# ElenaRyumina/AVCER

Hardware: AMD Instinct MI355X
Metric: clips/sec (224x224x16f + 2s@16kHz), full AV path: static CNN + LSTM + wav2vec2 audio model + fusion (higher is better)
Workload: dtype f16x3 (f16 MFMA on hi/lo-split f32 operands, f32 accumulate)

## Files before the change

avcer_amd/_lib.py:

```python
from __future__ import annotations

import ctypes as C
import os

from .build import LIB, source_hash

c_ctx = C.c_void_p
c_stream = C.c_void_p


class ConvDesc(C.Structure):
    _fields_ = [
        ("batch", C.c_int32), ("in_h", C.c_int32), ("in_w", C.c_int32),
        ("out_h", C.c_int32), ("out_w", C.c_int32),
        ("cin", C.c_int32), ("kh", C.c_int32), ("kw", C.c_int32),
        ("stride_h", C.c_int32), ("stride_w", C.c_int32), ("pad_h", C.c_int32), ("pad_w", C.c_int32),
        ("dil_h", C.c_int32), ("dil_w", C.c_int32),
        ("x_stride_b", C.c_int64), ("x_stride_h", C.c_int64), ("x_stride_w", C.c_int64),
        ("x_coff", C.c_int32), ("n", C.c_int32),
        ("y_ld", C.c_int64), ("y_coff", C.c_int32),
        ("r_ld", C.c_int64), ("r_coff", C.c_int32),
        ("act", C.c_int32), ("res_after_act", C.c_int32), ("groups", C.c_int32),
        ("x2_cin", C.c_int32), ("x2_coff", C.c_int32), ("x2_stride", C.c_int32),
        ("x2_stride_b", C.c_int64), ("x2_stride_h", C.c_int64), ("x2_stride_w", C.c_int64),
# ... 62 lines not shown
    "avcer_cam_render": (C.c_int, [c_ctx, C.c_void_p, C.c_void_p, C.c_void_p, C.c_void_p, C.c_int, C.c_void_p, C.c_double,
                                   C.c_void_p, c_stream]),
    "avcer_fuse": (C.c_int, [c_ctx, C.c_void_p, C.c_void_p, C.c_void_p, C.c_int, C.c_int, C.c_int, C.c_void_p,
                             C.c_void_p, C.c_int, C.c_int, C.c_void_p, C.c_void_p, c_stream]),
    "avcer_conv_gemm": (C.c_int, [c_ctx, C.POINTER(ConvDesc), C.c_int, C.c_void_p, C.c_void_p, C.c_void_p, C.c_void_p,
                                  C.c_void_p, C.c_void_p, c_stream]),
    "avcer_split_weights": (C.c_int, [c_ctx, C.c_void_p, C.c_void_p, C.c_size_t, c_stream]),
    "avcer_split_weight_rows": (C.c_int, [c_ctx, C.c_void_p, C.c_void_p, C.c_int, C.c_int, c_stream]),
    "avcer_weight_frags": (C.c_int, [c_ctx, C.c_void_p, C.c_void_p, C.c_int, C.c_int, c_stream]),
    "avcer_conv_gemm_dual": (C.c_int, [c_ctx, C.POINTER(ConvDesc), C.c_int, C.c_void_p, C.c_void_p, C.c_void_p, C.c_void_p,
                                       C.c_void_p, C.c_void_p, C.c_void_p, c_stream]),
    "avcer_face_nms": (C.c_int, [c_ctx, C.c_void_p, C.c_int, C.c_int, C.c_float, C.c_float, C.c_int, C.c_int, C.c_float,
                                 C.c_void_p, C.c_void_p, c_stream]),
    "avcer_bneck_chain": (C.c_int, [c_ctx, C.c_int, C.c_int, C.c_int, C.c_int, C.c_void_p, C.c_void_p, C.c_int, C.c_int] + [C.c_void_p] * 9 +
                          [c_stream]),
    "avcer_stem_pool": (C.c_int, [c_ctx, C.c_void_p, C.c_size_t, C.c_void_p, C.c_void_p, C.c_void_p, C.c_void_p, C.c_int, c_stream]),
    "avcer_stem_pool_u8": (C.c_int, [c_ctx, C.c_void_p, C.c_int, C.c_int, C.c_int, C.c_void_p, C.c_void_p, C.c_void_p, C.c_void_p,
                                     c_stream]),
    "avcer_attention": (C.c_int, [c_ctx, C.c_void_p, C.c_void_p, C.c_int, C.c_int, C.c_int, C.c_int, C.c_float, C.c_int, C.c_int,
                                  c_stream]),
    "avcer_measure_ceilings": (C.c_int, [c_ctx, C.POINTER(C.c_double), C.POINTER(C.c_double), c_stream]),
    "avcer_gemm_stats": (C.c_int, [c_ctx, C.POINTER(C.c_int64), C.POINTER(C.c_double), C.c_int]),
    "avcer_profile_enable": (C.c_int, [c_ctx, C.c_int]),
    "avcer_profile_read": (C.c_int, [c_ctx, C.POINTER(C.c_double), C.POINTER(C.c_int64)]),
    "avcer_profile_read_families": (C.c_int, [c_ctx, C.c_int, C.POINTER(C.c_double), C.POINTER(C.c_int64), C.POINTER(C.c_double),
                                              C.POINTER(C.c_double)]),
    "avcer_profile_read_launches": (C.c_int, [c_ctx, C.c_int64, C.c_void_p, C.c_void_p, C.c_void_p, C.c_void_p, C.c_void_p,
                                              C.POINTER(C.c_int64)]),
    "avcer_debug_tap": (C.c_int, [c_ctx, C.c_char_p, C.c_void_p, C.c_size_t]),
    "avcer_debug_tap_copied": (C.c_int64, [c_ctx]),
# ... 44 lines not shown
```

avcer_amd/csrc/api.hip:

```cpp
#include "common.h"
#include "split_dev.h"
#include "_source_hash.h"

#include <algorithm>
#include <cmath>
#include <new>

int set_err(avcer_ctx* ctx, int code, const char* fmt, ...) {
    if (ctx) {
        va_list ap;
        va_start(ap, fmt);
        vsnprintf(ctx->err, sizeof(ctx->err), fmt, ap);
        va_end(ap);
    }
    return code;
}

int ws_reserve(avcer_ctx* ctx, int slot, size_t bytes, void** out) {
    DevBuf& b = ctx->ws[slot];
    if (b.cap < bytes) {
        if (b.p) {
            HIP_TRY(ctx, hipDeviceSynchronize());
            HIP_TRY(ctx, hipFree(b.p));
            b.p = nullptr;
// ... 398 lines not shown
    }
    return AVCER_OK;
}
extern "C" int avcer_audio_num_classes(const avcer_ctx* ctx) { return ctx ? ctx->aud_classes : 0; }
extern "C" int avcer_audio_head_kind(const avcer_ctx* ctx) { return ctx && ctx->aud.loaded ? ctx->aud_head : 0; }

struct Trunk {
    void* X;
    void* pp[2];
    void* T1;
    void* T2;
    int h, w, cin;
    bool stride_last;
    bool w2_frags;
    const char* tap;
};

static void run_bneck_stage(Net& net, Trunk& t, int li, int b_begin, int b_end, int nb, void* last_out, const std::string& end_tap) {
    avcer_ctx* ctx = net.ctx;
    const std::string tap = t.tap;
    const int act = net.act.kind;
    const size_t es = net.act.es;
    const int planes = kStages[li][0], blocks = kStages[li][1];
    const int fused_from = li == 0 ? 0 : 1;
    for (int b = b_begin; b < b_end; ++b) {
        const int s = t.stride_last ? (b == blocks - 1 && li < 3 ? kStages[li + 1][2] : 1) : (b == 0 ? kStages[li][2] : 1);
        const int h = t.h, w = t.w, oh = (h - 1) / s + 1, ow = (w - 1) / s + 1;
        const long M = (long)nb * h * w;
        const std::string p = "l" + std::to_string(li + 1) + "." + std::to_string(b) + ".",
                          pn = "l" + std::to_string(li + 1) + "." + std::to_string(b + 1) + ".";
        void* dst = (b == b_end - 1 && last_out) ? last_out : (t.X == t.pp[0] ? t.pp[1] : t.pp[0]);
        const bool fused = net.x3 && li < 3 && b >= fused_from, chain = fused && li < 2, next = b + 1 < blocks;
        if (!fused || b == fused_from)
            net.gemm(conv2d_desc(nb, h, w, t.cin, 1, 1, 1, 0, planes, 1), p + "c1.w", net.F(p + "c1.s"), net.F(p + "c1.b"), t.X,
                     nullptr, t.T1, act, act);
        if (chain) {
            const bool first = b == 0;
            const Tensor *w2 = net.T(p + "c2.wf"), *w3 = net.T(first ? p + "c3d.w" : p + "c3.wf"),
                         *w1n = next ? net.T(pn + "c1.wf") : nullptr;
            if (net.err != AVCER_OK) return;
            if (!w2->x3 || !w3->x3 || (next && !w1n->x3)) {
                net.err = set_err(ctx, AVCER_ESTATE, "%s: split chain weights not prepared", p.c_str());
                return;
            }
            net.chk(launch_bneck(ctx, planes, nb, h, w, t.T1, t.X, first ? t.cin : 0, s, dst, next ? t.T2 : nullptr, w2->x3,
                                 net.F(p + "c2.b"), w3->x3, net.F(first ? p + "c3d.b" : p + "c3.b"), next ? w1n->x3 : nullptr,
                                 next ? net.F(pn + "c1.b") : nullptr, net.st, t.w2_frags ? w2->x3f : nullptr));
            if (ctx->tap_dst) {
                net.tap((tap + "chain_out:" + p).c_str(), dst, (size_t)nb * oh * ow * planes * 4 * es);
                if (next) net.tap((tap + "chain_t1n:" + p).c_str(), t.T2, (size_t)M * planes * es);
            }
            std::swap(t.T1, t.T2);
        } else {
            net.gemm(conv2d_desc(nb, h, w, planes, 3, 3, s, 1, planes, 1), p + "c2.w", net.F(p + "c2.s"), net.F(p + "c2.b"), t.T1,
                     nullptr, t.T2, act, act);
            avcer_conv_desc d3 = conv2d_desc(nb, oh, ow, planes, 1, 1, 1, 0, planes * 4, 1);
            if (fused && next && M <= kTailPairRows) {
                net.gemm(d3, p + "c3.wf", nullptr, net.F(p + "c3.b"), t.T2, t.X, dst, act, act);
                net.gemm(conv2d_desc(nb, h, w, planes * 4, 1, 1, 1, 0, planes, 1), pn + "c1.wf", nullptr, net.F(pn + "c1.b"), dst,
                         nullptr, t.T1, act, act);
            } else if (fused && next) {
                const Tensor *w3 = net.T(p + "c3.wf"), *w1n = net.T(pn + "c1.wf");
                if (net.err != AVCER_OK) return;
                if (!w3->x3 || !w1n->x3) {
                    net.err = set_err(ctx, AVCER_ESTATE, "%s: split tail weights not prepared", p.c_str());
// ... 770 lines not shown
                                    avcer_stream_t stream) {
    if (!ctx || !d || !x2) return AVCER_EINVAL;
    HIP_TRY(ctx, hipSetDevice(ctx->device));
    return launch_conv_gemm(ctx, *d, dtype, x, w, scale, bias, residual, y, (hipStream_t)stream, x2);
}

extern "C" int avcer_bneck_chain(avcer_ctx* ctx, int planes, int nb, int h, int w, const void* t1, const void* x, int ds_cin,
                                 int out_step, void* out, void* t1n, const void* w2, const float* b2, const void* w3, const float* b3,
                                 const void* w1n, const float* b1n, const void* w2_frags, avcer_stream_t stream) {
    if (!ctx) return AVCER_EINVAL;
    if (nb <= 0 || h <= 0 || w <= 0) return set_err(ctx, AVCER_EINVAL, "bneck_chain: bad geometry");
    HIP_TRY(ctx, hipSetDevice(ctx->device));
    return launch_bneck(ctx, planes, nb, h, w, t1, x, ds_cin, out_step, out, t1n, w2, b2, w3, b3, w1n, b1n, (hipStream_t)stream, w2_frags);
}

extern "C" int avcer_stem_pool(avcer_ctx* ctx, const void* planes_hi_lo, size_t plane_bytes, const void* w, const float* scale,
                               const float* bias, void* y, int n, avcer_stream_t stream) {
    if (!ctx) return AVCER_EINVAL;
    if (plane_bytes != (size_t)n * 230 * 230 * 4 * 2) return set_err(ctx, AVCER_EINVAL, "stem_pool: plane_bytes != n*230*230*4*2");
    HIP_TRY(ctx, hipSetDevice(ctx->device));
    return launch_stem_pool(ctx, planes_hi_lo, plane_bytes, w, scale, bias, y, n, (hipStream_t)stream);
}

extern "C" int avcer_stem_pool_u8(avcer_ctx* ctx, const uint8_t* frames, int n, int in_h, int in_w, const void* w, const float* scale,
                                  const float* shifts9, void* y, avcer_stream_t stream) {
    if (!ctx) return AVCER_EINVAL;
    HIP_TRY(ctx, hipSetDevice(ctx->device));
    return launch_stem_pool_u8(ctx, frames, in_h, in_w, w, scale, shifts9, y, n, (hipStream_t)stream);
}

// ... 46 lines not shown
```

avcer_amd/csrc/common.h:

```cpp
#pragma once

#include <hip/hip_runtime.h>

#include <cstdarg>
#include <cstdint>
#include <cstdio>
#include <cstring>
#include <map>
#include <string>
#include <vector>

#include "../../include/avcer_hip.h"
#include "arena.h"

typedef uint16_t bf16_t;

struct DevBuf {
    void* p = nullptr;
    size_t cap = 0;
};

enum { WS_STATIC = 0, WS_DYNAMIC = 1, WS_AUDIO = 2, WS_FACE = 3, WS_NMS = 4, WS_CEILINGS = 5, WS_STATIC_LANE1 = 6, WS_FACE_LANE1 = 7,
       WS_GRU = 8, WS_COUNT = 9 };

// ... 80 lines not shown
int launch_stem_pool(avcer_ctx* ctx, const void* planes, size_t plane_bytes, const void* w_x3, const float* scale,
                     const float* bias, void* y, int n, hipStream_t st);
int launch_stem_pool_u8(avcer_ctx* ctx, const uint8_t* frames, int in_h, int in_w, const void* w_x3, const float* scale,
                        const float* bias9, void* y, int n, hipStream_t st);
int launch_stem_pool_face(avcer_ctx* ctx, const uint8_t* frames, int h, int w, int rgb, const void* w_x3, const float* scale,
                          const float* bias, void* y, int n, hipStream_t st);
inline double grid_rounds(long tiles, long slots) {
    const long whole = tiles / slots, rest = tiles % slots;
    if (whole == 0) return 2 * tiles <= slots ? 0.62 : 1.0;
    const double f = (double)rest / (double)slots;
    return (double)whole + (rest == 0 ? 0.0 : (2 * rest <= slots ? 0.25 + 0.7 * f : 1.0));
}

int launch_bneck(avcer_ctx* ctx, int planes, int nb, int h, int w, const void* t1, const void* x, int ds_cin, int out_step,
                 void* out, void* t1n, const void* w2, const float* b2, const void* w3, const float* b3, const void* w1n,
                 const float* b1n, hipStream_t st, const void* w2_frags = nullptr);

int launch_bneck_tail(avcer_ctx* ctx, int planes, long M, const void* t2, const void* x, void* out, void* t1n, const void* w3,
                      const float* b3, const void* w1n, const float* b1n, hipStream_t st);

int launch_gru_layer(avcer_ctx* ctx, const float* xp, const void* w, int x3, const float* bhh, int n, int S, float* h_seq, void* h_sp,
                     hipStream_t st);

int measure_ceilings(avcer_ctx* ctx, double* mfma_bf16_tflops, double* hbm_copy_tbs, hipStream_t st);

int k_preprocess(avcer_ctx*, const uint8_t* frames, int n, int in_h, int in_w, void* out, int kind, hipStream_t);
int k_maxpool3s2(avcer_ctx*, const void* x, void* y, int n, int h, int w, int c, int oh, int ow, int kind, hipStream_t);
int k_avgpool_hw(avcer_ctx*, const void* x, float* y, void* y_sp32, int n, int hw, int c, int kind, hipStream_t);
int k_cam_maps(avcer_ctx*, const void* x, const float* probs, const float* h, const float* w1, const float* w2, float* g,
               float* cam, int n, int kind, hipStream_t);
int k_small_linear(avcer_ctx*, const float* x, const float* w, const float* b, float* logits, float* probs, int m,
// ... 38 lines not shown
```

avcer_amd/csrc/fused.hip:

```cpp
#include "common.h"
#include "gemm_dev.h"

#include <algorithm>

namespace {

__device__ __forceinline__ void mfma3(f32x4_t& acc, const spx8_t wh, const spx8_t wl, const spx8_t ah, const spx8_t al) {
    acc = mfma_sp(wl, ah, acc);
    acc = mfma_sp(wh, al, acc);
    acc = mfma_sp(wh, ah, acc);
}

template <int A, int B>
__device__ __forceinline__ void pin(f32x4_t (&acc)[A][B]) {
#pragma unroll
    for (int a = 0; a < A; ++a)
#pragma unroll
        for (int b = 0; b < B; ++b) asm volatile("" : "+v"(acc[a][b]));
}
template <int A>
__device__ __forceinline__ void pin(f32x4_t (&acc)[A]) {
#pragma unroll
    for (int a = 0; a < A; ++a) asm volatile("" : "+v"(acc[a]));
}
// ... 368 lines not shown
    char* OUT;
    char* T1N;
    const char* W2;
    const char* W2F;
    const char* W3;
    const char* W1N;
    const float *b2, *b3, *b1n;
    unsigned t1_bytes;
    int M, H, Wd;
    int OH, OW;
    unsigned* ovf;
    int nblocks;
};

template <int P, int BM, bool NEXT, int NQX, bool PATCH, int SUB = 1, bool T11 = false>
__global__ void __launch_bounds__(256, P == 64 ? 3 : 2) bneck_kernel(const BneckParams p) {
    static_assert(SUB == 1 || (SUB == 2 && !NEXT && NQX == 0 && !PATCH), "the strided form is the plain last block of a stage");
    static_assert(!T11 || (P == 64 && BM == 128 && !PATCH && SUB == 1), "the spatial-tile form serves planes 64 at full resolution");
    constexpr int NQ = P / 32;
    constexpr int NQT = NQ + NQX;
    constexpr int PSLOTS = PATCH ? (P == 64 ? 456 : 304) : 0;
    constexpr int T11_E = 11, T11_PW = T11_E + 2, T11_SLOTS = 176;
    constexpr int NT = BM / 64;
    constexpr int NG = 4 * P / 32;
    constexpr int TILE_A = (BM + P) * ROWB;
    constexpr int TILE_B = (32 * NQT + P) * ROWB;
    constexpr int PHASE_A = T11 ? NQ * T11_SLOTS * ROWB : (PATCH ? PSLOTS * ROWB + 2 * P * ROWB : 2 * TILE_A);
    constexpr int TILES = PHASE_A > 2 * TILE_B ? PHASE_A : 2 * TILE_B;
    constexpr int NBIAS = 6 * P;
    __shared__ __attribute__((aligned(16))) char smem[TILES + NBIAS * 4];
    float* sbias = reinterpret_cast<float*>(smem + TILES);
    for (int i = threadIdx.x; i < NBIAS; i += 256)
        sbias[i] = i < P ? p.b2[i] : (i < 2 * P ? (NEXT ? p.b1n[i - P] : 0.f) : p.b3[i - 2 * P]);
    const int wave = __builtin_amdgcn_readfirstlane((int)threadIdx.x >> 6);
    sp_flags_t ovm = 0;
    const int tid = threadIdx.x, lane = tid & 63;
    const int g = lane >> 4, l15 = lane & 15;
    const int lrow8 = lane >> 3, slot = lane & 7;
    const int blk = xcd_remap(blockIdx.x, gridDim.x);
    const int m_base = blk * BM;
    const int t11_b = T11 ? blk / 25 : 0, t11_y0 = T11 ? ((blk % 25) / 5) * T11_E : 0, t11_x0 = T11 ? (blk % 5) * T11_E : 0;
    auto row_pos = [&](int r, bool& ok) -> int {
        if constexpr (T11) {
            ok = r < T11_E * T11_E;
            const int rr = ok ? r : T11_E * T11_E - 1;
            const int ry = rr / T11_E, rx = rr - ry * T11_E;
            return (t11_b * 55 + t11_y0 + ry) * 55 + t11_x0 + rx;
        } else {
            const long m = (long)m_base + r;
            ok = m < p.M;
            return ok ? (int)m : 0;
        }
    };

    const float s2 = split_wmul(p.W2, P * 9 * P * 4), s3 = split_wmul(p.W3, 4 * P * (P + 32 * NQX) * 4);
    const float s1n = NEXT ? split_wmul(p.W1N, 4 * P * P * 4) : 1.f;
    (void)s1n;
    const auto t1rs = __builtin_amdgcn_make_buffer_rsrc(const_cast<char*>(p.T1), (short)0, (int)p.t1_bytes, 0x00020000);
    const auto w2rs = __builtin_amdgcn_make_buffer_rsrc(const_cast<char*>(p.W2), (short)0, P * 9 * P * 4, 0x00020000);
    const auto w3rs = __builtin_amdgcn_make_buffer_rsrc(const_cast<char*>(p.W3), (short)0, 4 * P * (P + 32 * NQX) * 4, 0x00020000);
    const auto w1rs = __builtin_amdgcn_make_buffer_rsrc(const_cast<char*>(NEXT ? p.W1N : p.W3), (short)0, 4 * P * P * 4, 0x00020000);

    constexpr int A_ISS = BM / 32;
    constexpr int W_ISS = P / 32;
    unsigned w_off[W_ISS];
#pragma unroll
    for (int j = 0; j < W_ISS; ++j) {
        const int row = wave * (W_ISS * 8) + j * 8 + lrow8;
        w_off[j] = (unsigned)((long)row * (9 * P * 4) + ((slot ^ swz_key(row)) << 4));
    }
    f32x4_t acc2[P / 16][NT];
#pragma unroll
    for (int i = 0; i < P / 16; ++i)
#pragma unroll
        for (int t = 0; t < NT; ++t) acc2[i][t] = f32x4_t{0};
    spx8_t t2h[NQ][NT], t2l[NQ][NT];
// ... 217 lines not shown
                al[t] = ldfrag(sa, row, 4 + g);
            }
#pragma unroll
            for (int i = 0; i < P / 16; ++i) {
                const spx8_t wh = ldfrag(sb, i * 16 + l15, g), wl = ldfrag(sb, i * 16 + l15, 4 + g);
#pragma unroll
                for (int t = 0; t < NT; ++t) mfma3(acc2[i][t], wh, wl, ah[t], al[t]);
            }
            pin(acc2);
            __syncthreads();
            cur ^= 1;
        }
    }
    }

    unsigned g3_off[NQT], g1_off[W_ISS];
#pragma unroll
    for (int j = 0; j < NQT; ++j) {
        const int row = wave * 8 + lrow8;
        g3_off[j] = (unsigned)((long)row * (NQT * ROWB) + j * ROWB + ((slot ^ swz_key(row)) << 4));
    }
#pragma unroll
    for (int j = 0; j < W_ISS; ++j) {
        const int row = wave * (W_ISS * 8) + j * 8 + lrow8;
        g1_off[j] = (unsigned)((long)row * (4 * P * 4) + ((slot ^ swz_key(row)) << 4));
    }
    auto issue_group = [&](int G) {
        char* base = smem + (G & 1) * TILE_B;
#pragma unroll
        for (int j = 0; j < NQT; ++j) dma16(w3rs, base + j * (32 * ROWB) + wave * 1024, g3_off[j], (unsigned)(G * 32 * NQT * ROWB));
        if constexpr (NEXT) {
#pragma unroll
            for (int j = 0; j < W_ISS; ++j)
                dma16(w1rs, base + NQT * (32 * ROWB) + wave * (W_ISS * 1024) + j * 1024, g1_off[j], (unsigned)(G * ROWB));
        }
    };
    issue_group(0);

    unsigned x_row[NT];
    unsigned o_row[SUB > 1 ? NT : 1];
    int m_row[NT];
    bool m_ok[NT];
#pragma unroll
    for (int t = 0; t < NT; ++t) {
        m_row[t] = row_pos(wave * (BM / 4) + t * 16 + l15, m_ok[t]);
        if constexpr (SUB == 1) {
            x_row[t] = (unsigned)(m_row[t] * (4L * P * 4) + 16 * g);
        } else {
            const int mm = m_row[t];
// ... 33 lines not shown
    load_res(1, rh[1], rl[1]);

#pragma unroll
    for (int q = 0; q < (T11 ? 0 : NQ); ++q) {
        const float4 b0 = *reinterpret_cast<const float4*>(sbias + 32 * q + 8 * g), b1 = *reinterpret_cast<const float4*>(sbias + 32 * q + 8 * g + 4);
#pragma unroll
        for (int t = 0; t < NT; ++t) {
            const f32x4_t lo4 = acc2[2 * q][t], hi4 = acc2[2 * q + 1][t];
            const float v[8] = {relu_nan(__builtin_fmaf(lo4[0], s2, b0.x)), relu_nan(__builtin_fmaf(lo4[1], s2, b0.y)),
                                relu_nan(__builtin_fmaf(lo4[2], s2, b0.z)), relu_nan(__builtin_fmaf(lo4[3], s2, b0.w)),
                                relu_nan(__builtin_fmaf(hi4[0], s2, b1.x)), relu_nan(__builtin_fmaf(hi4[1], s2, b1.y)),
                                relu_nan(__builtin_fmaf(hi4[2], s2, b1.z)), relu_nan(__builtin_fmaf(hi4[3], s2, b1.w))};
            split8v(v, t2h[q][t], t2l[q][t], ovm);
        }
    }
    f32x4_t acc1[NEXT ? P / 16 : 1][NT];
#pragma unroll
    for (int i = 0; i < (NEXT ? P / 16 : 1); ++i)
#pragma unroll
        for (int t = 0; t < NT; ++t) acc1[i][t] = f32x4_t{0};
    __syncthreads();

    auto group = [&](int G, uint4 (&h)[NT], uint4 (&l)[NT]) {
        if (G + 1 < NG) issue_group(G + 1);
        const char* w3t = smem + (G & 1) * TILE_B;
        const char* w1t = w3t + NQT * (32 * ROWB);
        f32x4_t acc3[2][NT];
#pragma unroll
        for (int tp = 0; tp < 2; ++tp)
#pragma unroll
            for (int t = 0; t < NT; ++t) acc3[tp][t] = f32x4_t{0};
#pragma unroll
        for (int q = 0; q < NQ; ++q)
// ... 2 lines not shown
                const spx8_t wh = ldfrag(w3t + q * (32 * ROWB), tp * 16 + l15, g), wl = ldfrag(w3t + q * (32 * ROWB), tp * 16 + l15, 4 + g);
#pragma unroll
                for (int t = 0; t < NT; ++t) mfma3(acc3[tp][t], wh, wl, t2h[q][t], t2l[q][t]);
            }
        if constexpr (NQX > 0) {
#pragma unroll
            for (int q = 0; q < NQX; ++q)
#pragma unroll
                for (int tp = 0; tp < 2; ++tp) {
                    const char* wt = w3t + (NQ + q) * (32 * ROWB);
                    const spx8_t wh = ldfrag(wt, tp * 16 + l15, g), wl = ldfrag(wt, tp * 16 + l15, 4 + g);
#pragma unroll
                    for (int t = 0; t < NT; ++t) mfma3(acc3[tp][t], wh, wl, xh[q][t], xl[q][t]);
                }
        }
        const float* bp = sbias + 2 * P + 32 * G + 8 * g;
        const float4 b0 = *reinterpret_cast<const float4*>(bp), b1 = *reinterpret_cast<const float4*>(bp + 4);
        spx8_t oh[NT], ol[NT];
#pragma unroll
        for (int t = 0; t < NT; ++t) {
            float r[8];
            unpack8(h[t], l[t], r);
            const f32x4_t lo4 = acc3[0][t], hi4 = acc3[1][t];
            const float v[8] = {relu_nan(__builtin_fmaf(lo4[0], s3, b0.x) + r[0]), relu_nan(__builtin_fmaf(lo4[1], s3, b0.y) + r[1]),
                                relu_nan(__builtin_fmaf(lo4[2], s3, b0.z) + r[2]), relu_nan(__builtin_fmaf(lo4[3], s3, b0.w) + r[3]),
                                relu_nan(__builtin_fmaf(hi4[0], s3, b1.x) + r[4]), relu_nan(__builtin_fmaf(hi4[1], s3, b1.y) + r[5]),
                                relu_nan(__builtin_fmaf(hi4[2], s3, b1.z) + r[6]), relu_nan(__builtin_fmaf(hi4[3], s3, b1.w) + r[7])};
            split8v(v, oh[t], ol[t], ovm);
            if (m_ok[t]) {
                char* yp = p.OUT + (size_t)(SUB == 1 ? x_row[t] : o_row[SUB > 1 ? t : 0]) + G * 128;
                *reinterpret_cast<spx8_t*>(yp) = oh[t];
                *reinterpret_cast<spx8_t*>(yp + 64) = ol[t];
            }
        }
        if (G + 2 < NG) load_res(G + 2, h, l);
        if constexpr (NEXT) {
#pragma unroll
            for (int i = 0; i < P / 16; ++i) {
                const spx8_t wh = ldfrag(w1t, i * 16 + l15, g), wl = ldfrag(w1t, i * 16 + l15, 4 + g);
#pragma unroll
                for (int t = 0; t < NT; ++t) mfma3(acc1[i][t], wh, wl, oh[t], ol[t]);
            }
            pin(acc1);
        }
        __syncthreads();
    };
    for (int G = 0; G < NG; G += 2) {
        group(G, rh[0], rl[0]);
        group(G + 1, rh[1], rl[1]);
    }

    if constexpr (NEXT) {
#pragma unroll
        for (int q = 0; q < NQ; ++q) {
            const float4 b0 = *reinterpret_cast<const float4*>(sbias + P + 32 * q + 8 * g), b1 = *reinterpret_cast<const float4*>(sbias + P + 32 * q + 8 * g + 4);
#pragma unroll
            for (int t = 0; t < NT; ++t) {
                const f32x4_t lo4 = acc1[2 * q][t], hi4 = acc1[2 * q + 1][t];
                const float v[8] = {relu_nan(__builtin_fmaf(lo4[0], s1n, b0.x)), relu_nan(__builtin_fmaf(lo4[1], s1n, b0.y)),
                                    relu_nan(__builtin_fmaf(lo4[2], s1n, b0.z)), relu_nan(__builtin_fmaf(lo4[3], s1n, b0.w)),
                                    relu_nan(__builtin_fmaf(hi4[0], s1n, b1.x)), relu_nan(__builtin_fmaf(hi4[1], s1n, b1.y)),
                                    relu_nan(__builtin_fmaf(hi4[2], s1n, b1.z)), relu_nan(__builtin_fmaf(hi4[3], s1n, b1.w))};
                spx8_t hi, lo;
                split8v(v, hi, lo, ovm);
                if (m_ok[t]) {
                    char* yp = p.T1N + (long)m_row[t] * (P * 4) + q * 128 + 16 * g;
                    *reinterpret_cast<spx8_t*>(yp) = hi;
                    *reinterpret_cast<spx8_t*>(yp + 64) = lo;
                }
            }
        }
    }
    sp_commit(p.ovf, ovm);
}


template <int P>
__global__ void __launch_bounds__(512, 2) bneck_tail2_kernel(const BneckParams p) {
    constexpr int NW = 8;
    constexpr int BM = 16 * NW;
    constexpr int NQ = P / 32;
// ... 227 lines not shown
    if (grid >= (1L << 31)) return set_err(ctx, AVCER_EINVAL, "stem_pool_face: %d frames of %d x %d are too many tiles for one launch", n, h, w);
    hipEvent_t ev0 = nullptr, ev1 = nullptr;
    const double flops = 2.0 * n * (double)p.oh * p.ow * 64 * 147;
    TRY(prof_begin(ctx, st, &ev0, &ev1, FAM_STEM, flops, (double)n * ((double)h * w * 3 + (double)p.mh * p.mw * 64 * 4), (long)n * p.oh * p.ow, 64, 147));
    stem_pool_u8_kernel<true><<<dim3((unsigned)grid), dim3(256), 0, st>>>(p);
    if (ev1) (void)hipEventRecord(ev1, st);
    hipError_t e = hipGetLastError();
    if (e != hipSuccess) return set_err(ctx, AVCER_EHIP, "stem_pool_face launch: %s", hipGetErrorString(e));
    ctx->gemm_launches += 1;
    ctx->gemm_flops += flops;
    return AVCER_OK;
}

int launch_bneck(avcer_ctx* ctx, int planes, int nb, int h, int w, const void* t1, const void* x, int ds_cin, int out_step,
                 void* out, void* t1n, const void* w2, const float* b2, const void* w3, const float* b3, const void* w1n,
                 const float* b1n, hipStream_t st, const void* w2_frags) {
    if (out_step != 1 && out_step != 2) return set_err(ctx, AVCER_EINVAL, "bneck: out_step %d (1 or 2)", out_step);
    if (out_step == 2 && (t1n || ds_cin)) return set_err(ctx, AVCER_EINVAL, "bneck: the strided form is the last block of a stage (no next conv1, no downsample)");
    const int oh = (h - 1) / out_step + 1, ow = (w - 1) / out_step + 1;
    const long M = (long)nb * oh * ow, M_in = (long)nb * h * w;
    if (!t1 || !x || !out || !w2 || !w3 || !b2 || !b3 || M <= 0)
        return set_err(ctx, AVCER_EINVAL, "bneck: bad arguments");
    if ((t1n != nullptr) != (w1n != nullptr) || (t1n && !b1n))
        return set_err(ctx, AVCER_EINVAL, "bneck: next-block conv1 needs weights, bias and an output");
    if (planes != 64 && planes != 128) return set_err(ctx, AVCER_EINVAL, "bneck: planes %d (64 or 128)", planes);
    if (ds_cin != 0 && !(ds_cin == 64 && planes == 64 && t1n))
        return set_err(ctx, AVCER_EINVAL, "bneck: the downsample form exists for planes 64 with a 64-channel input and a next conv1");
    const long x_bytes = M_in * (long)(ds_cin ? ds_cin : 4 * planes) * 4L, out_bytes = M * 4L * planes * 4L;
    if (M_in * planes * 4L >= (long)OOB || x_bytes >= (long)OOB || out_bytes >= (long)OOB)
        return set_err(ctx, AVCER_EINVAL, "bneck: %ld positions in, %ld out: a tensor of the pass reaches the 4 GiB offset range "
                                          "(at most %ld positions per call at planes %d)", M_in, M, ((long)OOB - 1) / (16L * planes), planes);
    BneckParams p;
    p.T1 = (const char*)t1; p.X = (const char*)x; p.OUT = (char*)out; p.T1N = (char*)t1n;
    p.W2 = (const char*)w2; p.W2F = (const char*)w2_frags; p.W3 = (const char*)w3; p.W1N = (const char*)w1n;
    p.b2 = b2; p.b3 = b3; p.b1n = b1n;
    p.t1_bytes = (unsigned)(M_in * planes * 4);
    p.M = (int)M; p.H = h; p.Wd = w; p.OH = oh; p.OW = ow; p.ovf = ctx->ovf;
    constexpr int BM = 128;
    const bool t11 = planes == 64 && h == 55 && w == 55 && out_step == 1 && t1n && w2_frags;
    p.nblocks = t11 ? nb * 25 : (int)((M + BM - 1) / BM);
    const int grid = p.nblocks;
    hipEvent_t ev0 = nullptr, ev1 = nullptr;
    {
        const double bytes = 4.0 * ((double)M_in * planes + (double)M * (ds_cin ? ds_cin : 4 * planes) + (double)M * 4 * planes +
                                    (t1n ? (double)M * planes : 0.0));
        TRY(prof_begin(ctx, st, &ev0, &ev1, FAM_CHAIN, 2.0 * (double)M * planes * (planes * (9.0 + 4.0 + (t1n ? 4.0 : 0.0)) + 4.0 * ds_cin), bytes, M,
                       4 * planes, planes));
    }
    const int rows_worst = (w - 1 + BM + w - 1) / w + 2 + 2;
    const bool patch = planes == 128 && (long)h * w >= BM && rows_worst * (w + 2) <= 304;
    if (out_step == 2) {
        if (planes == 64) bneck_kernel<64, BM, false, 0, false, 2><<<dim3(grid), dim3(256), 0, st>>>(p);
        else bneck_kernel<128, BM, false, 0, false, 2><<<dim3(grid), dim3(256), 0, st>>>(p);
    } else if (ds_cin) {
        if (t11) bneck_kernel<64, BM, true, 2, false, 1, true><<<dim3(grid), dim3(256), 0, st>>>(p);
        else bneck_kernel<64, BM, true, 2, false><<<dim3(grid), dim3(256), 0, st>>>(p);
    } else if (planes == 64) {
        if (t11) bneck_kernel<64, BM, true, 0, false, 1, true><<<dim3(grid), dim3(256), 0, st>>>(p);
        else if (t1n) bneck_kernel<64, BM, true, 0, false><<<dim3(grid), dim3(256), 0, st>>>(p);
        else bneck_kernel<64, BM, false, 0, false><<<dim3(grid), dim3(256), 0, st>>>(p);
    } else {
        if (t1n) {
            if (patch) bneck_kernel<128, BM, true, 0, true><<<dim3(grid), dim3(256), 0, st>>>(p);
            else bneck_kernel<128, BM, true, 0, false><<<dim3(grid), dim3(256), 0, st>>>(p);
        } else {
            if (patch) bneck_kernel<128, BM, false, 0, true><<<dim3(grid), dim3(256), 0, st>>>(p);
            else bneck_kernel<128, BM, false, 0, false><<<dim3(grid), dim3(256), 0, st>>>(p);
        }
    }
    if (ev1) (void)hipEventRecord(ev1, st);
    hipError_t e = hipGetLastError();
    if (e != hipSuccess) return set_err(ctx, AVCER_EHIP, "bneck launch: %s", hipGetErrorString(e));
    ctx->gemm_launches += 1;
    ctx->gemm_flops += 2.0 * (double)M * planes * (planes * (9.0 + 4.0 + (t1n ? 4.0 : 0.0)) + 4.0 * ds_cin);
    return AVCER_OK;
}

int launch_bneck_tail(avcer_ctx* ctx, int planes, long M, const void* t2, const void* x, void* out, void* t1n, const void* w3,
                      const float* b3, const void* w1n, const float* b1n, hipStream_t st) {
    if (!t2 || !x || !out || !t1n || !w3 || !b3 || !w1n || !b1n || M <= 0) return set_err(ctx, AVCER_EINVAL, "bneck_tail: bad arguments");
    if (planes != 256) return set_err(ctx, AVCER_EINVAL, "bneck_tail: planes %d (256)", planes);
    if (M * 4096L >= (1L << 32) - 4096) return set_err(ctx, AVCER_EINVAL, "bneck_tail: M=%ld exceeds the 4 GiB descriptor range", M);
    BneckParams p;
    memset(&p, 0, sizeof(p));
    p.T1 = (const char*)t2; p.X = (const char*)x; p.OUT = (char*)out; p.T1N = (char*)t1n;
    p.W3 = (const char*)w3; p.W1N = (const char*)w1n; p.b3 = b3; p.b1n = b1n;
    p.M = (int)M; p.ovf = ctx->ovf;
    hipEvent_t ev0 = nullptr, ev1 = nullptr;
    TRY(prof_begin(ctx, st, &ev0, &ev1, FAM_TAIL, 2.0 * (double)M * planes * planes * 8.0, 4.0 * (double)M * planes * 10.0, M, 4 * planes, planes));
// ... 42 lines not shown
```

avcer_amd/engine.py:

```python
from __future__ import annotations

import ctypes as C

import numpy as np
import torch

from . import _lib, packing
from ._lib import SPLIT_TRAILER, AvcerError, ConvDesc

MODE_FP32 = 0
MODE_BF16 = 1
MODE_F16X3 = 2
MODE_DEFAULT = MODE_F16X3
PAD_MODES = {"mean": 0, "constant": 1, "repeat": 2}


def _ptr(t):
    return None if t is None else C.c_void_p(t.data_ptr())


class Engine:
    def __init__(self, device: int = 0):
        if not torch.cuda.is_available():
            raise RuntimeError("avcer_amd needs a ROCm GPU (gfx950); there is no CPU path")
# ... 48 lines not shown
        if mode != MODE_F16X3:
            return call(mode)
        self.x3_overflow_clear()
        out = call(mode)
        if self.x3_overflow_count(reset=True):
            self.x3_fallbacks += 1
            out = call(MODE_FP32)
        return out

    def _load(self, fn, tensors):
        blob = packing.to_blob(tensors)
        buf = (C.c_char * len(blob)).from_buffer_copy(blob)
        self._check(fn(self.ctx, C.cast(buf, C.c_void_p), len(blob)))

    def load_static(self, state_dict):
        self._load(self.lib.avcer_load_static, packing.pack_static(state_dict))

    def load_dynamic(self, state_dict):
        self._load(self.lib.avcer_load_dynamic, packing.pack_dynamic(state_dict))

    def load_audio(self, state_dict):
        self._load(self.lib.avcer_load_audio, packing.pack_audio(state_dict))
        self.audio_classes = self.lib.avcer_audio_num_classes(self.ctx)

    @property
    def audio_head_kind(self) -> int:
        return int(self.lib.avcer_audio_head_kind(self.ctx))

    def load_face(self, state_dict):
        self._load(self.lib.avcer_load_face, packing.pack_face(state_dict))

# ... 373 lines not shown
        rows = self.split_weight_rows(w)
        out = torch.empty_like(rows)
        self._check(self.lib.avcer_weight_frags(self.ctx, _ptr(rows), _ptr(out), int(w.shape[0]), int(w.shape[1]), self._stream()))
        return out

    def conv_gemm_dual(self, desc: ConvDesc, dtype: int, x, x2, w, scale, bias, residual, y):
        self._check(self.lib.avcer_conv_gemm_dual(self.ctx, C.byref(desc), dtype, _ptr(x), _ptr(x2), _ptr(w), _ptr(scale),
                                                  _ptr(bias), _ptr(residual), _ptr(y), self._stream()))

    def bneck_chain(self, planes: int, nb: int, h: int, w: int, t1, x, out, t1n, w2, b2, w3, b3, w1n=None, b1n=None, ds_cin: int = 0,
                    out_step: int = 1, w2_frags=None):
        self._check(self.lib.avcer_bneck_chain(self.ctx, planes, nb, h, w, _ptr(t1), _ptr(x), int(ds_cin), int(out_step), _ptr(out),
                                               _ptr(t1n), _ptr(w2), _ptr(b2), _ptr(w3), _ptr(b3), _ptr(w1n), _ptr(b1n),
                                               _ptr(w2_frags), self._stream()))

    def attention(self, qkv, out, n: int, s: int, heads: int, head_dim: int, scale: float, in_kind: int, out_kind: int):
        self._check(self.lib.avcer_attention(self.ctx, _ptr(qkv), _ptr(out), n, s, heads, head_dim, float(scale), in_kind,
                                             out_kind, self._stream()))

    def measure_ceilings(self):
        a, b = C.c_double(0.0), C.c_double(0.0)
        self._check(self.lib.avcer_measure_ceilings(self.ctx, C.byref(a), C.byref(b), self._stream()))
        return a.value, b.value

    def stem_pool(self, planes_hi_lo, w_split, scale, bias, n: int):
        planes = self._dev(planes_hi_lo, torch.int16)
        if tuple(planes.shape) != (2, n, 230, 230, 4):
            raise ValueError("stem_pool: planes [2, n, 230, 230, 4] int16 (fp16 bits)")
        y = torch.empty(n, 55, 55, 128, dtype=torch.int16, device=self.device)
        self._check(self.lib.avcer_stem_pool(self.ctx, _ptr(planes), n * 230 * 230 * 4 * 2, _ptr(w_split), _ptr(scale), _ptr(bias),
# ... 16 lines not shown
```

avcer_amd/packing.py:

```python
from __future__ import annotations

import struct
from collections import OrderedDict

import numpy as np

STATIC_BN_EPS = 1e-3
AUDIO_BN_EPS = 1e-5
RESNET_STAGES = ((64, 3, 1), (128, 4, 2), (256, 6, 2), (512, 3, 2))
PE_ROWS = 256


def _np(v) -> np.ndarray:
    if hasattr(v, "detach"):
        v = v.detach().cpu().numpy()
    return np.asarray(v)


def _f32(v) -> np.ndarray:
    return np.ascontiguousarray(_np(v), dtype=np.float32)


def _unwrap(sd):
    if "model_state_dict" in sd and not hasattr(sd["model_state_dict"], "shape"):
# ... 22 lines not shown


PIXEL_MEANS = (91.4953, 103.8827, 131.0912)


def stem_border_shifts(w, scale, shift) -> np.ndarray:
    w = np.asarray(w, np.float64)
    mu = np.asarray(PIXEL_MEANS, np.float64)
    valid = (slice(2, 7), slice(0, 7), slice(0, 6))
    out = np.empty((9, w.shape[0]), np.float64)
    for ry, vy in enumerate(valid):
        for rx, vx in enumerate(valid):
            c = np.einsum("ocyx,c->o", w[:, :, vy, vx], mu)
            out[3 * ry + rx] = np.asarray(shift, np.float64) - np.asarray(scale, np.float64) * c
    return out.astype(np.float32)


def _fold_fused_weights(out, li: int, blocks: int) -> None:
    if li <= 2:
        for b in range(0 if li == 1 else 1, blocks):
            head = b == (0 if li == 1 else 1)
            for i in (1, 2, 3):
                if (i == 1 and head) or (i == 3 and b == 0):
                    continue
                k = f"l{li}.{b}.c{i}"
                out[k + ".wf"] = np.ascontiguousarray(out[k + ".w"] * out[k + ".s"][:, None])
    if li == 3:
        for b in range(1, blocks - 1):
            for k in (f"l{li}.{b}.c3", f"l{li}.{b + 1}.c1"):
                out[k + ".wf"] = np.ascontiguousarray(out[k + ".w"] * out[k + ".s"][:, None])
# ... 199 lines not shown
```

include/avcer_hip.h:

```cpp
#ifndef AVCER_HIP_H
#define AVCER_HIP_H

#include <stddef.h>
#include <stdint.h>

#ifdef __cplusplus
extern "C" {
#endif

typedef struct avcer_ctx avcer_ctx;
typedef void* avcer_stream_t;

enum {
    AVCER_OK = 0,
    AVCER_EINVAL = -1,
    AVCER_ENOMEM = -2,
    AVCER_EHIP = -3,
    AVCER_ESTATE = -4,
    AVCER_EFORMAT = -5
};

enum {
    AVCER_MODE_FP32 = 0,
    AVCER_MODE_BF16 = 1,
// ... 110 lines not shown
    int64_t x2_stride_b, x2_stride_h, x2_stride_w;
    int32_t tile_n;
    int32_t r_sub, r_h, r_w;
    int32_t tile_m;
} avcer_conv_desc;

int avcer_conv_gemm(avcer_ctx* ctx, const avcer_conv_desc* d, int dtype, const void* x, const void* w,
                    const float* scale, const float* bias, const void* residual, void* y, avcer_stream_t stream);

int avcer_conv_gemm_dual(avcer_ctx* ctx, const avcer_conv_desc* d, int dtype, const void* x, const void* x2, const void* w,
                         const float* scale, const float* bias, const void* residual, void* y, avcer_stream_t stream);

int avcer_bneck_chain(avcer_ctx* ctx, int planes, int nb, int h, int w, const void* t1, const void* x, int ds_cin, int out_step,
                      void* out, void* t1n, const void* w2, const float* b2, const void* w3, const float* b3, const void* w1n,
                      const float* b1n, const void* w2_frags, avcer_stream_t stream);
int avcer_stem_pool(avcer_ctx* ctx, const void* planes_hi_lo, size_t plane_bytes, const void* w, const float* scale,
                    const float* bias, void* y, int n, avcer_stream_t stream);
int avcer_stem_pool_u8(avcer_ctx* ctx, const uint8_t* frames, int n, int in_h, int in_w, const void* w, const float* scale,
                       const float* shifts9, void* y, avcer_stream_t stream);

int avcer_split_weights(avcer_ctx* ctx, const float* w, void* out, size_t numel, avcer_stream_t stream);

#define AVCER_SPLIT_TRAILER 256

int avcer_split_weight_rows(avcer_ctx* ctx, const float* w, void* out, int n, int k, avcer_stream_t stream);

int avcer_weight_frags(avcer_ctx* ctx, const void* rows, void* out, int n, int k, avcer_stream_t stream);

int avcer_gru_layer(avcer_ctx* ctx, const float* xp, const float* w_hh, const float* b_hh, int n, int s, int h, int mode,
                    float* h_seq, avcer_stream_t stream);
// ... 32 lines not shown
```

Measured before the change: 2175.

## Fuse next stage's conv1 into the strided last bottleneck block of stage one

The strided last block of the planes-64 stage now also computes the next stage's 1x1 conv1 (128 output channels) from its output tile, writing T1 for stage two directly. The trunk flag t1_ready lets stage two skip its standalone conv1 GEMM launch, and a packing step folds the scale into l2.0.c1 weights. This removes one kernel launch and one full read of the stage output. In exchange the fused kernel holds larger accumulators and shared-memory tiles, and its occupancy bound drops to 2 blocks per CU.

```diff
diff --git a/avcer_amd/_lib.py b/avcer_amd/_lib.py
--- a/avcer_amd/_lib.py
+++ b/avcer_amd/_lib.py
@@ -100,6 +100,7 @@
                                  C.c_void_p, C.c_void_p, c_stream]),
     "avcer_bneck_chain": (C.c_int, [c_ctx, C.c_int, C.c_int, C.c_int, C.c_int, C.c_void_p, C.c_void_p, C.c_int, C.c_int] + [C.c_void_p] * 9 +
                           [c_stream]),
+    "avcer_bneck_chain_entry": (C.c_int, [c_ctx, C.c_int, C.c_int, C.c_int, C.c_int] + [C.c_void_p] * 10 + [c_stream]),
     "avcer_stem_pool": (C.c_int, [c_ctx, C.c_void_p, C.c_size_t, C.c_void_p, C.c_void_p, C.c_void_p, C.c_void_p, C.c_int, c_stream]),
     "avcer_stem_pool_u8": (C.c_int, [c_ctx, C.c_void_p, C.c_int, C.c_int, C.c_int, C.c_void_p, C.c_void_p, C.c_void_p, C.c_void_p,
                                      c_stream]),
diff --git a/avcer_amd/csrc/api.hip b/avcer_amd/csrc/api.hip
--- a/avcer_amd/csrc/api.hip
+++ b/avcer_amd/csrc/api.hip
@@ -436,6 +436,7 @@
     bool stride_last;
     bool w2_frags;
     const char* tap;
+    bool t1_ready = false;
 };
 
 static void run_bneck_stage(Net& net, Trunk& t, int li, int b_begin, int b_end, int nb, void* last_out, const std::string& end_tap) {
@@ -453,24 +454,31 @@
                           pn = "l" + std::to_string(li + 1) + "." + std::to_string(b + 1) + ".";
         void* dst = (b == b_end - 1 && last_out) ? last_out : (t.X == t.pp[0] ? t.pp[1] : t.pp[0]);
         const bool fused = net.x3 && li < 3 && b >= fused_from, chain = fused && li < 2, next = b + 1 < blocks;
-        if (!fused || b == fused_from)
+        if (t.t1_ready) t.t1_ready = false;
+        else if (!fused || b == fused_from)
             net.gemm(conv2d_desc(nb, h, w, t.cin, 1, 1, 1, 0, planes, 1), p + "c1.w", net.F(p + "c1.s"), net.F(p + "c1.b"), t.X,
                      nullptr, t.T1, act, act);
         if (chain) {
             const bool first = b == 0;
+            const bool entry = !next && t.stride_last && s == 2 && planes == 64;
+            const std::string pe = entry ? "l" + std::to_string(li + 2) + ".0." : pn;
+            const bool next1 = next || entry;
             const Tensor *w2 = net.T(p + "c2.wf"), *w3 = net.T(first ? p + "c3d.w" : p + "c3.wf"),
-                         *w1n = next ? net.T(pn + "c1.wf") : nullptr;
+                         *w1n = next1 ? net.T(pe + "c1.wf") : nullptr;
             if (net.err != AVCER_OK) return;
-            if (!w2->x3 || !w3->x3 || (next && !w1n->x3)) {
+            if (!w2->x3 || !w3->x3 || (next1 && !w1n->x3)) {
                 net.err = set_err(ctx, AVCER_ESTATE, "%s: split chain weights not prepared", p.c_str());
                 return;
             }
-            net.chk(launch_bneck(ctx, planes, nb, h, w, t.T1, t.X, first ? t.cin : 0, s, dst, next ? t.T2 : nullptr, w2->x3,
-                                 net.F(p + "c2.b"), w3->x3, net.F(first ? p + "c3d.b" : p + "c3.b"), next ? w1n->x3 : nullptr,
-                                 next ? net.F(pn + "c1.b") : nullptr, net.st, t.w2_frags ? w2->x3f : nullptr));
+            net.chk(launch_bneck(ctx, planes, nb, h, w, t.T1, t.X, first ? t.cin : 0, s, dst, next1 ? t.T2 : nullptr, w2->x3,
+                                 net.F(p + "c2.b"), w3->x3, net.F(first ? p + "c3d.b" : p + "c3.b"), next1 ? w1n->x3 : nullptr,
+                                 next1 ? net.F(pe + "c1.b") : nullptr, net.st, t.w2_frags ? w2->x3f : nullptr,
+                                 entry ? 2 * planes : planes));
+            t.t1_ready = entry;
             if (ctx->tap_dst) {
                 net.tap((tap + "chain_out:" + p).c_str(), dst, (size_t)nb * oh * ow * planes * 4 * es);
                 if (next) net.tap((tap + "chain_t1n:" + p).c_str(), t.T2, (size_t)M * planes * es);
+                if (entry) net.tap((tap + "chain_t1n:" + p).c_str(), t.T2, (size_t)nb * oh * ow * 2 * planes * es);
             }
             std::swap(t.T1, t.T2);
         } else {
@@ -1271,6 +1279,16 @@
     return launch_bneck(ctx, planes, nb, h, w, t1, x, ds_cin, out_step, out, t1n, w2, b2, w3, b3, w1n, b1n, (hipStream_t)stream, w2_frags);
 }
 
+extern "C" int avcer_bneck_chain_entry(avcer_ctx* ctx, int planes, int nb, int h, int w, const void* t1, const void* x, void* out,
+                                       void* t1n, const void* w2, const float* b2, const void* w3, const float* b3, const void* w1n,
+                                       const float* b1n, avcer_stream_t stream) {
+    if (!ctx) return AVCER_EINVAL;
+    if (nb <= 0 || h <= 0 || w <= 0) return set_err(ctx, AVCER_EINVAL, "bneck_chain_entry: bad geometry");
+    if (!t1n || !w1n || !b1n) return set_err(ctx, AVCER_EINVAL, "bneck_chain_entry: the next stage's conv1 needs weights, bias and an output");
+    HIP_TRY(ctx, hipSetDevice(ctx->device));
+    return launch_bneck(ctx, planes, nb, h, w, t1, x, 0, 2, out, t1n, w2, b2, w3, b3, w1n, b1n, (hipStream_t)stream, nullptr, 2 * planes);
+}
+
 extern "C" int avcer_stem_pool(avcer_ctx* ctx, const void* planes_hi_lo, size_t plane_bytes, const void* w, const float* scale,
                                const float* bias, void* y, int n, avcer_stream_t stream) {
     if (!ctx) return AVCER_EINVAL;
diff --git a/avcer_amd/csrc/common.h b/avcer_amd/csrc/common.h
--- a/avcer_amd/csrc/common.h
+++ b/avcer_amd/csrc/common.h
@@ -118,7 +118,7 @@
 
 int launch_bneck(avcer_ctx* ctx, int planes, int nb, int h, int w, const void* t1, const void* x, int ds_cin, int out_step,
                  void* out, void* t1n, const void* w2, const float* b2, const void* w3, const float* b3, const void* w1n,
-                 const float* b1n, hipStream_t st, const void* w2_frags = nullptr);
+                 const float* b1n, hipStream_t st, const void* w2_frags = nullptr, int next_planes = 0);
 
 int launch_bneck_tail(avcer_ctx* ctx, int planes, long M, const void* t2, const void* x, void* out, void* t1n, const void* w3,
                       const float* b3, const void* w1n, const float* b1n, hipStream_t st);
diff --git a/avcer_amd/csrc/fused.hip b/avcer_amd/csrc/fused.hip
--- a/avcer_amd/csrc/fused.hip
+++ b/avcer_amd/csrc/fused.hip
@@ -406,8 +406,9 @@
 };
 
 template <int P, int BM, bool NEXT, int NQX, bool PATCH, int SUB = 1, bool T11 = false>
-__global__ void __launch_bounds__(256, P == 64 ? 3 : 2) bneck_kernel(const BneckParams p) {
-    static_assert(SUB == 1 || (SUB == 2 && !NEXT && NQX == 0 && !PATCH), "the strided form is the plain last block of a stage");
+__global__ void __launch_bounds__(256, P == 64 ? (NEXT && SUB == 2 ? 2 : 3) : 2) bneck_kernel(const BneckParams p) {
+    static_assert(SUB == 1 || (SUB == 2 && NQX == 0 && !PATCH), "the strided form is the last block of a stage");
+    static_assert(!(SUB == 2 && NEXT) || P == 64, "the next stage's conv1 behind the strided form: planes 64 only (see above)");
     static_assert(!T11 || (P == 64 && BM == 128 && !PATCH && SUB == 1), "the spatial-tile form serves planes 64 at full resolution");
     constexpr int NQ = P / 32;
     constexpr int NQT = NQ + NQX;
@@ -415,15 +416,16 @@
     constexpr int T11_E = 11, T11_PW = T11_E + 2, T11_SLOTS = 176;
     constexpr int NT = BM / 64;
     constexpr int NG = 4 * P / 32;
+    constexpr int N1 = NEXT && SUB == 2 ? 2 * P : P;
     constexpr int TILE_A = (BM + P) * ROWB;
-    constexpr int TILE_B = (32 * NQT + P) * ROWB;
+    constexpr int TILE_B = (32 * NQT + N1) * ROWB;
     constexpr int PHASE_A = T11 ? NQ * T11_SLOTS * ROWB : (PATCH ? PSLOTS * ROWB + 2 * P * ROWB : 2 * TILE_A);
     constexpr int TILES = PHASE_A > 2 * TILE_B ? PHASE_A : 2 * TILE_B;
-    constexpr int NBIAS = 6 * P;
+    constexpr int NBIAS = 5 * P + N1, B3OFF = P + N1;
     __shared__ __attribute__((aligned(16))) char smem[TILES + NBIAS * 4];
     float* sbias = reinterpret_cast<float*>(smem + TILES);
     for (int i = threadIdx.x; i < NBIAS; i += 256)
-        sbias[i] = i < P ? p.b2[i] : (i < 2 * P ? (NEXT ? p.b1n[i - P] : 0.f) : p.b3[i - 2 * P]);
+        sbias[i] = i < P ? p.b2[i] : (i < B3OFF ? (NEXT ? p.b1n[i - P] : 0.f) : p.b3[i - B3OFF]);
     const int wave = __builtin_amdgcn_readfirstlane((int)threadIdx.x >> 6);
     sp_flags_t ovm = 0;
     const int tid = threadIdx.x, lane = tid & 63;
@@ -446,12 +448,12 @@
     };
 
     const float s2 = split_wmul(p.W2, P * 9 * P * 4), s3 = split_wmul(p.W3, 4 * P * (P + 32 * NQX) * 4);
-    const float s1n = NEXT ? split_wmul(p.W1N, 4 * P * P * 4) : 1.f;
+    const float s1n = NEXT ? split_wmul(p.W1N, N1 * 4 * P * 4) : 1.f;
     (void)s1n;
     const auto t1rs = __builtin_amdgcn_make_buffer_rsrc(const_cast<char*>(p.T1), (short)0, (int)p.t1_bytes, 0x00020000);
     const auto w2rs = __builtin_amdgcn_make_buffer_rsrc(const_cast<char*>(p.W2), (short)0, P * 9 * P * 4, 0x00020000);
     const auto w3rs = __builtin_amdgcn_make_buffer_rsrc(const_cast<char*>(p.W3), (short)0, 4 * P * (P + 32 * NQX) * 4, 0x00020000);
-    const auto w1rs = __builtin_amdgcn_make_buffer_rsrc(const_cast<char*>(NEXT ? p.W1N : p.W3), (short)0, 4 * P * P * 4, 0x00020000);
+    const auto w1rs = __builtin_amdgcn_make_buffer_rsrc(const_cast<char*>(NEXT ? p.W1N : p.W3), (short)0, NEXT ? N1 * 4 * P * 4 : 4 * P * P * 4, 0x00020000);
 
     constexpr int A_ISS = BM / 32;
     constexpr int W_ISS = P / 32;
@@ -699,15 +701,16 @@
     }
     }
 
-    unsigned g3_off[NQT], g1_off[W_ISS];
+    constexpr int W1_ISS = N1 / 32;
+    unsigned g3_off[NQT], g1_off[W1_ISS];
 #pragma unroll
     for (int j = 0; j < NQT; ++j) {
         const int row = wave * 8 + lrow8;
         g3_off[j] = (unsigned)((long)row * (NQT * ROWB) + j * ROWB + ((slot ^ swz_key(row)) << 4));
     }
 #pragma unroll
-    for (int j = 0; j < W_ISS; ++j) {
-        const int row = wave * (W_ISS * 8) + j * 8 + lrow8;
+    for (int j = 0; j < W1_ISS; ++j) {
+        const int row = wave * (W1_ISS * 8) + j * 8 + lrow8;
         g1_off[j] = (unsigned)((long)row * (4 * P * 4) + ((slot ^ swz_key(row)) << 4));
     }
     auto issue_group = [&](int G) {
@@ -716,8 +719,8 @@
         for (int j = 0; j < NQT; ++j) dma16(w3rs, base + j * (32 * ROWB) + wave * 1024, g3_off[j], (unsigned)(G * 32 * NQT * ROWB));
         if constexpr (NEXT) {
 #pragma unroll
-            for (int j = 0; j < W_ISS; ++j)
-                dma16(w1rs, base + NQT * (32 * ROWB) + wave * (W_ISS * 1024) + j * 1024, g1_off[j], (unsigned)(G * ROWB));
+            for (int j = 0; j < W1_ISS; ++j)
+                dma16(w1rs, base + NQT * (32 * ROWB) + wave * (W1_ISS * 1024) + j * 1024, g1_off[j], (unsigned)(G * ROWB));
         }
     };
     issue_group(0);
@@ -781,9 +784,9 @@
             split8v(v, t2h[q][t], t2l[q][t], ovm);
         }
     }
-    f32x4_t acc1[NEXT ? P / 16 : 1][NT];
-#pragma unroll
-    for (int i = 0; i < (NEXT ? P / 16 : 1); ++i)
+    f32x4_t acc1[NEXT ? N1 / 16 : 1][NT];
+#pragma unroll
+    for (int i = 0; i < (NEXT ? N1 / 16 : 1); ++i)
 #pragma unroll
         for (int t = 0; t < NT; ++t) acc1[i][t] = f32x4_t{0};
     __syncthreads();
@@ -816,7 +819,7 @@
                     for (int t = 0; t < NT; ++t) mfma3(acc3[tp][t], wh, wl, xh[q][t], xl[q][t]);
                 }
         }
-        const float* bp = sbias + 2 * P + 32 * G + 8 * g;
+        const float* bp = sbias + B3OFF + 32 * G + 8 * g;
         const float4 b0 = *reinterpret_cast<const float4*>(bp), b1 = *reinterpret_cast<const float4*>(bp + 4);
         spx8_t oh[NT], ol[NT];
 #pragma unroll
@@ -838,7 +841,7 @@
         if (G + 2 < NG) load_res(G + 2, h, l);
         if constexpr (NEXT) {
 #pragma unroll
-            for (int i = 0; i < P / 16; ++i) {
+            for (int i = 0; i < N1 / 16; ++i) {
                 const spx8_t wh = ldfrag(w1t, i * 16 + l15, g), wl = ldfrag(w1t, i * 16 + l15, 4 + g);
 #pragma unroll
                 for (int t = 0; t < NT; ++t) mfma3(acc1[i][t], wh, wl, oh[t], ol[t]);
@@ -854,7 +857,7 @@
 
     if constexpr (NEXT) {
 #pragma unroll
-        for (int q = 0; q < NQ; ++q) {
+        for (int q = 0; q < N1 / 32; ++q) {
             const float4 b0 = *reinterpret_cast<const float4*>(sbias + P + 32 * q + 8 * g), b1 = *reinterpret_cast<const float4*>(sbias + P + 32 * q + 8 * g + 4);
 #pragma unroll
             for (int t = 0; t < NT; ++t) {
@@ -866,7 +869,7 @@
                 spx8_t hi, lo;
                 split8v(v, hi, lo, ovm);
                 if (m_ok[t]) {
-                    char* yp = p.T1N + (long)m_row[t] * (P * 4) + q * 128 + 16 * g;
+                    char* yp = p.T1N + (long)m_row[t] * (N1 * 4) + q * 128 + 16 * g;
                     *reinterpret_cast<spx8_t*>(yp) = hi;
                     *reinterpret_cast<spx8_t*>(yp + 64) = lo;
                 }
@@ -1124,9 +1127,15 @@
 
 int launch_bneck(avcer_ctx* ctx, int planes, int nb, int h, int w, const void* t1, const void* x, int ds_cin, int out_step,
                  void* out, void* t1n, const void* w2, const float* b2, const void* w3, const float* b3, const void* w1n,
-                 const float* b1n, hipStream_t st, const void* w2_frags) {
+                 const float* b1n, hipStream_t st, const void* w2_frags, int next_planes) {
     if (out_step != 1 && out_step != 2) return set_err(ctx, AVCER_EINVAL, "bneck: out_step %d (1 or 2)", out_step);
-    if (out_step == 2 && (t1n || ds_cin)) return set_err(ctx, AVCER_EINVAL, "bneck: the strided form is the last block of a stage (no next conv1, no downsample)");
+    if (out_step == 2 && ds_cin) return set_err(ctx, AVCER_EINVAL, "bneck: the strided form is the last block of a stage (no downsample)");
+    if (t1n && next_planes != (out_step == 2 ? 2 * planes : planes) && !(out_step == 1 && next_planes == 0))
+        return set_err(ctx, AVCER_EINVAL, "bneck: the strided form is the last block of a stage: a conv1 behind it is the next stage's, of %d "
+                                          "channels (avcer_bneck_chain_entry); inside a stage it has %d (got %d)", 2 * planes, planes, next_planes);
+    if (t1n && out_step == 2 && planes != 64)
+        return set_err(ctx, AVCER_EINVAL, "bneck: the strided form runs the next stage's conv1 at planes 64 only (planes %d)", planes);
+    const int n1 = t1n ? (out_step == 2 ? 2 * planes : planes) : 0;
     const int oh = (h - 1) / out_step + 1, ow = (w - 1) / out_step + 1;
     const long M = (long)nb * oh * ow, M_in = (long)nb * h * w;
     if (!t1 || !x || !out || !w2 || !w3 || !b2 || !b3 || M <= 0)
@@ -1153,14 +1162,15 @@
     hipEvent_t ev0 = nullptr, ev1 = nullptr;
     {
         const double bytes = 4.0 * ((double)M_in * planes + (double)M * (ds_cin ? ds_cin : 4 * planes) + (double)M * 4 * planes +
-                                    (t1n ? (double)M * planes : 0.0));
-        TRY(prof_begin(ctx, st, &ev0, &ev1, FAM_CHAIN, 2.0 * (double)M * planes * (planes * (9.0 + 4.0 + (t1n ? 4.0 : 0.0)) + 4.0 * ds_cin), bytes, M,
+                                    (double)M * n1);
+        TRY(prof_begin(ctx, st, &ev0, &ev1, FAM_CHAIN, 2.0 * (double)M * planes * (planes * (9.0 + 4.0) + 4.0 * n1 + 4.0 * ds_cin), bytes, M,
                        4 * planes, planes));
     }
     const int rows_worst = (w - 1 + BM + w - 1) / w + 2 + 2;
     const bool patch = planes == 128 && (long)h * w >= BM && rows_worst * (w + 2) <= 304;
     if (out_step == 2) {
-        if (planes == 64) bneck_kernel<64, BM, false, 0, false, 2><<<dim3(grid), dim3(256), 0, st>>>(p);
+        if (planes == 64 && t1n) bneck_kernel<64, BM, true, 0, false, 2><<<dim3(grid), dim3(256), 0, st>>>(p);
+        else if (planes == 64) bneck_kernel<64, BM, false, 0, false, 2><<<dim3(grid), dim3(256), 0, st>>>(p);
         else bneck_kernel<128, BM, false, 0, false, 2><<<dim3(grid), dim3(256), 0, st>>>(p);
     } else if (ds_cin) {
         if (t11) bneck_kernel<64, BM, true, 2, false, 1, true><<<dim3(grid), dim3(256), 0, st>>>(p);
@@ -1182,7 +1192,7 @@
     hipError_t e = hipGetLastError();
     if (e != hipSuccess) return set_err(ctx, AVCER_EHIP, "bneck launch: %s", hipGetErrorString(e));
     ctx->gemm_launches += 1;
-    ctx->gemm_flops += 2.0 * (double)M * planes * (planes * (9.0 + 4.0 + (t1n ? 4.0 : 0.0)) + 4.0 * ds_cin);
+    ctx->gemm_flops += 2.0 * (double)M * planes * (planes * (9.0 + 4.0) + 4.0 * n1 + 4.0 * ds_cin);
     return AVCER_OK;
 }
 
diff --git a/avcer_amd/engine.py b/avcer_amd/engine.py
--- a/avcer_amd/engine.py
+++ b/avcer_amd/engine.py
@@ -86,7 +86,7 @@
         self._check(fn(self.ctx, C.cast(buf, C.c_void_p), len(blob)))
 
     def load_static(self, state_dict):
-        self._load(self.lib.avcer_load_static, packing.pack_static(state_dict))
+        self._load(self.lib.avcer_load_static, packing.fold_stage_entry_weights(packing.pack_static(state_dict)))
 
     def load_dynamic(self, state_dict):
         self._load(self.lib.avcer_load_dynamic, packing.pack_dynamic(state_dict))
@@ -490,6 +490,10 @@
                                                _ptr(t1n), _ptr(w2), _ptr(b2), _ptr(w3), _ptr(b3), _ptr(w1n), _ptr(b1n),
                                                _ptr(w2_frags), self._stream()))
 
+    def bneck_chain_entry(self, planes: int, nb: int, h: int, w: int, t1, x, out, t1n, w2, b2, w3, b3, w1n, b1n):
+        self._check(self.lib.avcer_bneck_chain_entry(self.ctx, planes, nb, h, w, _ptr(t1), _ptr(x), _ptr(out), _ptr(t1n), _ptr(w2),
+                                                     _ptr(b2), _ptr(w3), _ptr(b3), _ptr(w1n), _ptr(b1n), self._stream()))
+
     def attention(self, qkv, out, n: int, s: int, heads: int, head_dim: int, scale: float, in_kind: int, out_kind: int):
         self._check(self.lib.avcer_attention(self.ctx, _ptr(qkv), _ptr(out), n, s, heads, head_dim, float(scale), in_kind,
                                              out_kind, self._stream()))
diff --git a/avcer_amd/packing.py b/avcer_amd/packing.py
--- a/avcer_amd/packing.py
+++ b/avcer_amd/packing.py
@@ -60,6 +60,12 @@
             c = np.einsum("ocyx,c->o", w[:, :, vy, vx], mu)
             out[3 * ry + rx] = np.asarray(shift, np.float64) - np.asarray(scale, np.float64) * c
     return out.astype(np.float32)
+
+
+def fold_stage_entry_weights(out):
+    k = "l2.0.c1"
+    out[k + ".wf"] = np.ascontiguousarray(out[k + ".w"] * out[k + ".s"][:, None])
+    return out
 
 
 def _fold_fused_weights(out, li: int, blocks: int) -> None:
diff --git a/include/avcer_hip.h b/include/avcer_hip.h
--- a/include/avcer_hip.h
+++ b/include/avcer_hip.h
@@ -148,6 +148,9 @@
 int avcer_bneck_chain(avcer_ctx* ctx, int planes, int nb, int h, int w, const void* t1, const void* x, int ds_cin, int out_step,
                       void* out, void* t1n, const void* w2, const float* b2, const void* w3, const float* b3, const void* w1n,
                       const float* b1n, const void* w2_frags, avcer_stream_t stream);
+int avcer_bneck_chain_entry(avcer_ctx* ctx, int planes, int nb, int h, int w, const void* t1, const void* x, void* out, void* t1n,
+                            const void* w2, const float* b2, const void* w3, const float* b3, const void* w1n, const float* b1n,
+                            avcer_stream_t stream);
 int avcer_stem_pool(avcer_ctx* ctx, const void* planes_hi_lo, size_t plane_bytes, const void* w, const float* scale,
                     const float* bias, void* y, int n, avcer_stream_t stream);
 int avcer_stem_pool_u8(avcer_ctx* ctx, const uint8_t* frames, int n, int in_h, int in_w, const void* w, const float* scale,
```

After: 2185 (median of 6 runs). About the same (+0.4%).
